# yanielc/medical-vision-textural-bias

Hardware: AMD Instinct MI355X
Metric: BraTS 4ch 240^3 vols/sec filtered+train-step @1/2/4/8 GPU; filter HBM GB/s (higher is better)
Workload: dtype f32

## Files before the change

### medical-vision-textural-bias_amd/csrc/conv_small.hip

```cpp
#include <hip/hip_runtime.h>

#include <cstdlib>

#include "texbias.h"
#include "kernels.h"

namespace {

constexpr int NT = 256;
constexpr int ROWS = 6;
constexpr int WPT = 4;
constexpr int kSeg = 3;

template <int CI, int CO>
__global__ __launch_bounds__(NT) void k_conv3d_small(const float* __restrict__ x, const float* __restrict__ wt,
                                                     const float* __restrict__ bias, float* __restrict__ y, int D,
                                                     int H, int W, int XP, int nhb) {
  extern __shared__ __attribute__((aligned(16))) float xs[];
  static_assert(WPT == 4, "the input reads are one float4 + one float2");
  float* ws = xs + CI * 3 * (ROWS + 2) * XP;
  const int tid = (int)threadIdx.x;
  for (int i = tid; i < CO * CI * 27; i += NT) ws[i] = wt[i];
  const int hb = (int)blockIdx.x % nhb, z = (int)blockIdx.x / nhb, n = (int)blockIdx.y;
  const int h0 = hb * ROWS;
  const int64_t plane = (int64_t)H * W, vol = (int64_t)D * plane;
  constexpr int NR = CI * 3 * (ROWS + 2);
  const int lane = tid & 63, wave = __builtin_amdgcn_readfirstlane(tid >> 6);
  static_assert(NR % (NT / 64) == 0, "rows deal evenly to the waves");
#pragma unroll
  for (int row = wave; row < NR; row += NT / 64) {
    const int ci = row / (3 * (ROWS + 2)), rem = row - ci * (3 * (ROWS + 2));
    const int tz = rem / (ROWS + 2), r = rem - tz * (ROWS + 2);
    const int zi = z + tz - 1, hi = h0 + r - 1;
    const bool ok = zi >= 0 && zi < D && hi >= 0 && hi < H;
    const float* src = x + ((int64_t)n * CI + ci) * vol + (ok ? (int64_t)zi * plane + (int64_t)hi * W : 0) - 1;
    float* dst = xs + row * XP;
#pragma unroll
    for (int sg = 0; sg < kSeg; ++sg) {
      const int col = lane + 64 * sg;
      const bool in = ok && col >= 1 && col <= W;
      const float v = src[in ? col : 1];
      if (col < XP) dst[col] = in ? v : 0.f;
    }
  }
  __syncthreads();
  const int tpr = (W + WPT - 1) / WPT;
  const int r = tid / tpr, w0 = (tid - r * tpr) * WPT;
  if (r >= ROWS || h0 + r >= H) return;
  float acc[CO][WPT];
#pragma unroll
  for (int co = 0; co < CO; ++co) {
    const float b = bias ? bias[co] : 0.f;
#pragma unroll
    for (int k = 0; k < WPT; ++k) acc[co][k] = b;
  }
#pragma unroll 1
  for (int ct = 0; ct < CI * 3; ++ct) {
    const int ci = ct / 3, tz = ct - 3 * ci;
    {
#pragma unroll
      for (int ty = 0; ty < 3; ++ty) {
        const float* src = xs + (ct * (ROWS + 2) + r + ty) * XP + w0;
        const float4 v4 = *reinterpret_cast<const float4*>(src);
        const float2 v2 = *reinterpret_cast<const float2*>(src + 4);
        const float v[WPT + 2] = {v4.x, v4.y, v4.z, v4.w, v2.x, v2.y};
#pragma unroll
        for (int co = 0; co < CO; ++co) {
#pragma unroll
          for (int tx = 0; tx < 3; ++tx) {
            const float wv = ws[(((co * CI + ci) * 3 + tz) * 3 + ty) * 3 + tx];
#pragma unroll
            for (int k = 0; k < WPT; ++k) acc[co][k] = fmaf(wv, v[k + tx], acc[co][k]);
          }
        }
      }
    }
  }
  const int h = h0 + r;
#pragma unroll
  for (int co = 0; co < CO; ++co) {
    float* dst = y + ((int64_t)n * CO + co) * vol + (int64_t)z * plane + (int64_t)h * W + w0;
#pragma unroll
    for (int k = 0; k < WPT; ++k)
      if (w0 + k < W) dst[k] = acc[co][k];
  }
}

typedef __attribute__((address_space(1))) const void* gptr_t;
typedef __attribute__((address_space(3))) void* lptr_t;
#ifndef TB_SMALL_ZB
#define TB_SMALL_ZB 8
#endif
constexpr int ZB = TB_SMALL_ZB;

#ifndef TB_SMALL_SW
#define TB_SMALL_SW 1
#endif
typedef const __attribute__((address_space(4))) float* cfloat_sp;

template <int CI, int CO, bool ADD = false, int U = 1>
__global__ __launch_bounds__(NT) void k_conv3d_small_z(const float* __restrict__ x, const float* __restrict__ wt,
                                                       const float* __restrict__ bias, float* __restrict__ y, int D,
                                                       int H, int W, int XP, int nhb, const float* __restrict__ add) {
  extern __shared__ __attribute__((aligned(16))) float xs[];
  constexpr int RS = ROWS + 2, NR = CI * RS;
  const int slot_f = CI * RS * XP;
  float* ws = xs + 4 * slot_f;
  const int tid = (int)threadIdx.x, lane = tid & 63, wave = __builtin_amdgcn_readfirstlane(tid >> 6);
  for (int i = tid; i < 4 * slot_f; i += NT) xs[i] = 0.f;
  for (int i = tid; i < CO * CI * 27; i += NT) ws[i] = wt[i];
  const int hb = (int)blockIdx.x % nhb, z0 = ((int)blockIdx.x / nhb) * ZB, n = (int)blockIdx.y;
  const int h0 = hb * ROWS;
  const int64_t plane = (int64_t)H * W, vol = (int64_t)D * plane;
  __syncthreads();
  auto stage = [&](int zi) {
    float* sl = xs + ((zi - z0 + 1) & 3) * slot_f;
    for (int row = wave; row < NR; row += NT / 64) {
      const int ci = row / RS, r = row - ci * RS, hi = h0 + r - 1;
      float* dst = sl + row * XP + 1;
      if (zi >= 0 && zi < D && hi >= 0 && hi < H) {
        const float* src = x + ((int64_t)n * CI + ci) * vol + (int64_t)zi * plane + (int64_t)hi * W;
#pragma unroll
        for (int sg = 0; sg < kSeg; ++sg) {
          const int c = lane + 64 * sg;
          if (c < W) __builtin_amdgcn_global_load_lds((gptr_t)(src + c), (lptr_t)(dst + 64 * sg), 4, 0, 0);
        }
      } else {
#pragma unroll
        for (int sg = 0; sg < kSeg; ++sg) {
          const int c = lane + 64 * sg;
          if (c < W) dst[c] = 0.f;
        }
      }
    }
  };
  stage(z0 - 1);
  stage(z0);
  stage(z0 + 1);
  __builtin_amdgcn_s_waitcnt(0);
  __syncthreads();
  const int tpr = (W + WPT - 1) / WPT;
  const int r = tid / tpr, w0 = (tid - r * tpr) * WPT;
  const bool act = r < ROWS && h0 + r < H;
  const int zend = z0 + ZB < D ? z0 + ZB : D;
  const int h = h0 + r;
  float prev[CO][WPT], padd[CO][WPT];
  auto put = [&](int zp) {
#pragma unroll
    for (int co = 0; co < CO; ++co) {
      const int64_t o = ((int64_t)n * CO + co) * vol + (int64_t)zp * plane + (int64_t)h * W + w0;
#pragma unroll
      for (int k = 0; k < WPT; ++k)
        if (w0 + k < W) y[o + k] = ADD ? prev[co][k] + padd[co][k] : prev[co][k];
    }
  };
  for (int z = z0; z < zend; ++z) {
    if (z + 2 < zend + 1) stage(z + 2);
    if (act) {
      if (z > z0) put(z - 1);
      if (ADD) {
#pragma unroll
        for (int co = 0; co < CO; ++co) {
          const int64_t o = ((int64_t)n * CO + co) * vol + (int64_t)z * plane + (int64_t)h * W + w0;
#pragma unroll
          for (int k = 0; k < WPT; ++k) padd[co][k] = w0 + k < W ? add[o + k] : 0.f;
        }
      }
      float acc[CO][WPT];
#pragma unroll
      for (int co = 0; co < CO; ++co) {
        const float b = bias ? bias[co] : 0.f;
#pragma unroll
        for (int k = 0; k < WPT; ++k) acc[co][k] = b;
      }
#pragma unroll U
      for (int ct = 0; ct < CI * 3; ++ct) {
        const int ci = ct / 3, tz = ct - 3 * ci;
        const float* base = xs + ((z - z0 + tz) & 3) * slot_f + (ci * RS + r) * XP + w0;
#pragma unroll
        for (int ty = 0; ty < 3; ++ty) {
          const float* src = base + ty * XP;
          const float4 v4 = *reinterpret_cast<const float4*>(src);
          const float2 v2 = *reinterpret_cast<const float2*>(src + 4);
          const float v[WPT + 2] = {v4.x, v4.y, v4.z, v4.w, v2.x, v2.y};
#pragma unroll
          for (int co = 0; co < CO; ++co) {
#pragma unroll
            for (int tx = 0; tx < 3; ++tx) {
              const int wi = (((co * CI + ci) * 3 + tz) * 3 + ty) * 3 + tx;
              const float wv = TB_SMALL_SW ? ((cfloat_sp)wt)[wi] : ws[wi];
#pragma unroll
              for (int k = 0; k < WPT; ++k) acc[co][k] = fmaf(wv, v[k + tx], acc[co][k]);
            }
          }
        }
      }
#pragma unroll
      for (int co = 0; co < CO; ++co)
#pragma unroll
        for (int k = 0; k < WPT; ++k) prev[co][k] = acc[co][k];
    }
    __builtin_amdgcn_s_waitcnt(0);
    __syncthreads();
  }
  if (act && zend > z0) put(zend - 1);
}

__global__ __launch_bounds__(256) void k_add_inplace(float* __restrict__ y, const float* __restrict__ a, int64_t n) {
  for (int64_t i = (int64_t)blockIdx.x * 256 + threadIdx.x; i < n; i += (int64_t)gridDim.x * 256) y[i] += a[i];
}

template <int CI, int CO>
int launch(const float* x, const float* w, const float* b, const float* add, float* y, int N, int D, int H, int W,
           hipStream_t st) {
  const int XP = (W + 2 + WPT + 3) / 4 * 4;
  const size_t lds = sizeof(float) * ((size_t)CI * 3 * (ROWS + 2) * XP + CO * CI * 27);
  if ((W + WPT - 1) / WPT * ROWS > NT || lds > 65536 || XP > 64 * kSeg) return TB_ERR_UNSUPPORTED_SIZE;
  const int nhb = (H + ROWS - 1) / ROWS;
  const size_t lds_z = sizeof(float) * ((size_t)4 * CI * (ROWS + 2) * XP + CO * CI * 27);
  if (lds_z <= 65536 * 2) {
    void (*kern)(const float*, const float*, const float*, float*, int, int, int, int, int, const float*) =
        add ? k_conv3d_small_z<CI, CO, true, 3> : k_conv3d_small_z<CI, CO, false, 3>;
    if (tb::allow_full_lds(kern) != hipSuccess) return TB_ERR_HIP;
    hipLaunchKernelGGL(kern, dim3((unsigned)(nhb * ((D + ZB - 1) / ZB)), (unsigned)N), dim3(NT), lds_z, st, x, w, b, y,
                       D, H, W, XP, nhb, add);
    return hipGetLastError() == hipSuccess ? TB_OK : TB_ERR_HIP;
  }
  hipLaunchKernelGGL((k_conv3d_small<CI, CO>), dim3((unsigned)(nhb * D), (unsigned)N), dim3(NT), lds, st, x, w, b, y,
                     D, H, W, XP, nhb);
  if (add) {
    const int64_t n = (int64_t)N * CO * D * H * W;
    hipLaunchKernelGGL(k_add_inplace, dim3((unsigned)((n + 1023) / 1024 < 8192 ? (n + 1023) / 1024 : 8192)), dim3(256),
                       0, st, y, add, n);
  }
  return hipGetLastError() == hipSuccess ? TB_OK : TB_ERR_HIP;
}

}

int tb_conv3d_small_f32(const float* x, const float* w, const float* b, float* y, int N, int Cin, int Cout, int D,
                        int H, int W, void* stream) {
  return tb_conv3d_small_add_f32(x, w, b, nullptr, y, N, Cin, Cout, D, H, W, stream);
}

int tb_conv3d_small_add_f32(const float* x, const float* w, const float* b, const float* add, float* y, int N, int Cin,
                            int Cout, int D, int H, int W, void* stream) {
  if (!x || !w || !y || N < 1 || D < 1 || H < 1 || W < 1 || N > 65535) return TB_ERR_INVALID_ARG;
  if (Cin < 1 || Cin > 4 || Cout < 1 || Cout > 4) return TB_ERR_UNSUPPORTED_SIZE;
  hipStream_t st = reinterpret_cast<hipStream_t>(stream);
#define TB_CASE(ci, co) \
  if (Cin == ci && Cout == co) return launch<ci, co>(x, w, b, add, y, N, D, H, W, st);
#define TB_ROW(ci) TB_CASE(ci, 1) TB_CASE(ci, 2) TB_CASE(ci, 3) TB_CASE(ci, 4)
  TB_ROW(1) TB_ROW(2) TB_ROW(3) TB_ROW(4)
#undef TB_ROW
#undef TB_CASE
  return TB_ERR_UNSUPPORTED_SIZE;
}
```

### medical-vision-textural-bias_amd/csrc/conv_up.hip

```cpp
#include <hip/hip_runtime.h>

#include <cstdlib>

#include "num_cu.h"
#include "texbias.h"

namespace {

typedef float f2v __attribute__((ext_vector_type(2)));
typedef float f32x4 __attribute__((ext_vector_type(4)));
typedef const __attribute__((address_space(4))) float* cfloat_p;
typedef const __attribute__((address_space(4))) f2v* cf2v_p;

struct S2Args {
  const float* in;
  const float* K;
  const float* bias;
  float* out;
  int Do, Ho, Wo, Di, Hi, Wi;
  int ZS, zlen, nyb;
  int PX, RR;
};

template <int CIN, int MOUT, int TY, int WV, int NTH = 256>
__global__ __launch_bounds__(NTH) void k_conv_s2_fewin(S2Args a) {
  static_assert(MOUT % 2 == 0, "packed output pairs");
  constexpr int NHALF = NTH / 256, MP = MOUT / 2 / NHALF;
  constexpr int NR = 2 * TY + 1;
  extern __shared__ __attribute__((aligned(16))) float smem[];
  const int tid = (int)threadIdx.x;
  constexpr int PX = 4 * WV + 12, SS = CIN * NR * PX;
  float* ring = smem;
  for (int i = tid; i < 3 * SS; i += NTH) ring[i] = 0.f;
  int b = (int)blockIdx.x;
  const int zs = b % a.ZS;
  b /= a.ZS;
  const int yb = b % a.nyb, n = b / a.nyb;
  const int y0 = yb * TY;
  const int z0 = zs * a.zlen, z1 = min(a.Do, z0 + a.zlen);
  const int Di = a.Di, Hi = a.Hi, Wi = a.Wi;
  const int64_t iplane = (int64_t)Hi * Wi, iplane4 = iplane / 4;
  const float4* inb = reinterpret_cast<const float4*>(a.in + (int64_t)n * CIN * Di * iplane);
  const int W4 = Wi >> 2;
  constexpr int NL = (CIN * NR * WV + NTH - 1) / NTH;
  int gof[NL], lof[NL];
#pragma unroll
  for (int j = 0; j < NL; ++j) {
    const int i = tid + NTH * j;
    const int q = i % W4, t = i / W4, r = t % NR, c = t / NR;
    const int yi = 2 * y0 - 1 + r;
    const bool ok = c < CIN && yi >= 0 && yi < Hi;
    gof[j] = ok ? (int)((int64_t)c * Di * iplane4 + ((int64_t)yi * Wi + 4 * q) / 4) : -1;
    lof[j] = (c * NR + r) * PX + 4 + 4 * q;
  }
  float4 ra[NL], rb[NL];
  auto load = [&](int zi, float4 (&r)[NL]) {
    const bool in = zi >= 0 && zi < Di;
    const float4* src = inb + (int64_t)(in ? zi : 0) * iplane4;
#pragma unroll
    for (int j = 0; j < NL; ++j) {
      r[j] = src[gof[j] < 0 ? 0 : gof[j]];
    }
  };
  auto store = [&](int zi, const float4 (&r)[NL]) {
    float* d = ring + ((zi + 3) % 3) * SS;
    const bool in = zi >= 0 && zi < Di;
#pragma unroll
    for (int j = 0; j < NL; ++j)
      if (gof[j] >= 0) *reinterpret_cast<float4*>(d + lof[j]) = in ? r[j] : make_float4(0.f, 0.f, 0.f, 0.f);
  };
  __syncthreads();
  load(2 * z0 - 1, ra);
  store(2 * z0 - 1, ra);
  load(2 * z0, ra);
  load(2 * z0 + 1, rb);
  const int pt = tid & 255, mh = __builtin_amdgcn_readfirstlane(tid >> 8);
  const int Wo = a.Wo, oy = pt / Wo, ox = pt - oy * Wo;
  const bool act = oy < TY && y0 + oy < a.Ho;
  const int roff = (2 * oy) * PX + 2 * ox + 3;
  f2v bias2[MP];
#pragma unroll
  for (int mm = 0; mm < MP; ++mm) {
    const int m = mh * MP + mm;
    bias2[mm] = a.bias ? f2v{a.bias[2 * m], a.bias[2 * m + 1]} : f2v{0.f, 0.f};
  }
  const int64_t oplane = (int64_t)a.Ho * Wo;
  float* outb = a.out + (int64_t)n * MOUT * a.Do * oplane + (int64_t)(y0 + oy) * Wo + ox;
  constexpr bool LATE = NTH == 256;
  f2v pend[MP];
  auto put = [&](int zp) {
    float* o = outb + (int64_t)zp * oplane;
#pragma unroll
    for (int mm = 0; mm < MP; ++mm) {
      const int m = mh * MP + mm;
      o[(int64_t)(2 * m) * a.Do * oplane] = pend[mm].x;
      o[(int64_t)(2 * m + 1) * a.Do * oplane] = pend[mm].y;
    }
  };
  for (int z = z0; z < z1; ++z) {
    store(2 * z, ra);
    store(2 * z + 1, rb);
    __syncthreads();
    if (LATE || z + 1 < z1) {
      load(2 * z + 2, ra);
      load(2 * z + 3, rb);
    }
    if (LATE && act && z > z0) put(z - 1);
    if (act) {
      float v[CIN * 27];
#pragma unroll
      for (int tz = 0; tz < 3; ++tz) {
        const float* sl = ring + ((2 * z - 1 + tz + 3) % 3) * SS + roff;
#pragma unroll
        for (int c = 0; c < CIN; ++c)
#pragma unroll
          for (int ty = 0; ty < 3; ++ty)
#pragma unroll
            for (int tx = 0; tx < 3; ++tx) v[c * 27 + tz * 9 + ty * 3 + tx] = sl[(c * NR + ty) * PX + tx];
      }
      const cf2v_p kp = (cf2v_p)(cfloat_p)a.K;
#pragma unroll
      for (int mm = 0; mm < MP; ++mm) {
        const int m = mh * MP + mm;
        f2v acc = bias2[mm];
#pragma unroll
        for (int k = 0; k < CIN * 27; ++k) acc = __builtin_elementwise_fma(f2v{v[k], v[k]}, kp[m * CIN * 27 + k], acc);
        if (LATE) {
          pend[mm] = acc;
        } else {
          float* o = outb + (int64_t)z * oplane;
          o[(int64_t)(2 * m) * a.Do * oplane] = acc.x;
          o[(int64_t)(2 * m + 1) * a.Do * oplane] = acc.y;
        }
      }
    }
    __syncthreads();
  }
  if (LATE && act && z1 > z0) put(z1 - 1);
}

struct TArgs {
  const float* x;
  const float* W;
  const float* bias;
  float* y;
  int Cin, Di, Hi, Wi;
  int ZS, zlen, nyb;
  int PX, CS;
};

template <int MO, int TY, int WV, int NTH = 256, int U = 1>
__global__ __launch_bounds__(NTH) void k_convT_fewout(TArgs a) {
  extern __shared__ __attribute__((aligned(16))) float smem[];
  const int tid = (int)threadIdx.x;
  constexpr int PX = 4 * WV + 8, CS = (TY + 1) * PX;
  const int Cin = a.Cin, SS = Cin * CS;
  float* ring = smem;
  for (int i = tid; i < 2 * SS; i += NTH) ring[i] = 0.f;
  const cfloat_p wg = (cfloat_p)a.W;
  int b = (int)blockIdx.x;
  const int zs = b % a.ZS;
  b /= a.ZS;
  const int yb = b % a.nyb, n = b / a.nyb;
  const int y0 = yb * TY;
  const int Di = a.Di, Hi = a.Hi, Wi = a.Wi;
  const int z0 = zs * a.zlen, z1 = min(Di, z0 + a.zlen);
  const int64_t iplane = (int64_t)Hi * Wi, iplane4 = iplane / 4;
  const float4* xb = reinterpret_cast<const float4*>(a.x + (int64_t)n * Cin * Di * iplane);
  const int W4 = Wi >> 2;
  constexpr int NL = (32 * (TY + 1) * WV + NTH - 1) / NTH;
  const int nitem = Cin * (TY + 1) * W4;
  int gof[NL], lof[NL];
#pragma unroll
  for (int j = 0; j < NL; ++j) {
    const int i = tid + NTH * j;
    const int q = i % W4, t = i / W4, r = t % (TY + 1), c = t / (TY + 1);
    const int yi = y0 + r;
    const bool ok = i < nitem && yi < Hi;
    gof[j] = ok ? (int)((int64_t)c * Di * iplane4 + ((int64_t)yi * Wi + 4 * q) / 4) : -1;
    lof[j] = c * CS + r * PX + 4 + 4 * q;
  }
  float4 rg[NL];
  auto load = [&](int zi) {
    const bool in = zi < Di;
    const float4* src = xb + (int64_t)(in ? zi : 0) * iplane4;
#pragma unroll
    for (int j = 0; j < NL; ++j) {
      rg[j] = src[gof[j] < 0 ? 0 : gof[j]];
    }
  };
  auto store = [&](int zi) {
    float* d = ring + (zi & 1) * SS;
    const bool in = zi < Di;
#pragma unroll
    for (int j = 0; j < NL; ++j)
      if (gof[j] >= 0) *reinterpret_cast<float4*>(d + lof[j]) = in ? rg[j] : make_float4(0.f, 0.f, 0.f, 0.f);
  };
  __syncthreads();
  load(z0);
  store(z0);
  load(z0 + 1);
  const int jy = tid / Wi, jx = tid - jy * Wi;
  const bool act = jy < TY && y0 + jy < Hi;
  const int roff = jy * PX + jx + 4;
  const int Ho = 2 * Hi, Wo = 2 * Wi, Do = 2 * Di;
  const int64_t oplane = (int64_t)Ho * Wo;
  float bia[MO];
#pragma unroll
  for (int m = 0; m < MO; ++m) bia[m] = a.bias ? a.bias[m] : 0.f;
  float* yb0 = a.y + (int64_t)n * MO * Do * oplane + (int64_t)(2 * (y0 + jy)) * Wo + 2 * jx;
  for (int z = z0; z < z1; ++z) {
    store(z + 1);
    __syncthreads();
    if (z + 1 < z1) load(z + 2);
    float acc[MO][2][2][2];
#pragma unroll
    for (int m = 0; m < MO; ++m)
#pragma unroll
      for (int p = 0; p < 8; ++p) acc[m][p >> 2][(p >> 1) & 1][p & 1] = bia[m];
    if (act) {
      const float* s0 = ring + (z & 1) * SS + roff;
      const float* s1 = ring + ((z + 1) & 1) * SS + roff;
#pragma unroll U
      for (int c = 0; c < Cin; ++c) {
        float v[2][2][2];
        v[0][0][0] = s0[c * CS];
        v[0][0][1] = s0[c * CS + 1];
        v[0][1][0] = s0[c * CS + PX];
        v[0][1][1] = s0[c * CS + PX + 1];
        v[1][0][0] = s1[c * CS];
        v[1][0][1] = s1[c * CS + 1];
        v[1][1][0] = s1[c * CS + PX];
        v[1][1][1] = s1[c * CS + PX + 1];
        const cfloat_p wc = wg + c * MO * 27;
#pragma unroll
        for (int m = 0; m < MO; ++m) {
          const cfloat_p wk = wc + m * 27;
#pragma unroll
          for (int pz = 0; pz < 2; ++pz)
#pragma unroll
            for (int py = 0; py < 2; ++py)
#pragma unroll
              for (int px = 0; px < 2; ++px) {
                float s = acc[m][pz][py][px];
#pragma unroll
                for (int dz = 0; dz <= pz; ++dz)
#pragma unroll
                  for (int dy = 0; dy <= py; ++dy)
#pragma unroll
                    for (int dx = 0; dx <= px; ++dx) {
                      const int tz = pz ? (dz ? 0 : 2) : 1, ty = py ? (dy ? 0 : 2) : 1, tx = px ? (dx ? 0 : 2) : 1;
                      s = fmaf(v[dz][dy][dx], wk[tz * 9 + ty * 3 + tx], s);
                    }
                acc[m][pz][py][px] = s;
              }
        }
      }
#pragma unroll
      for (int m = 0; m < MO; ++m)
#pragma unroll
        for (int pz = 0; pz < 2; ++pz)
#pragma unroll
          for (int py = 0; py < 2; ++py) {
            float* o = yb0 + ((int64_t)m * Do + 2 * z + pz) * oplane + (int64_t)py * Wo;
            *reinterpret_cast<float2*>(o) = make_float2(acc[m][pz][py][0], acc[m][pz][py][1]);
          }
    }
    __syncthreads();
  }
}

int zseg(int D, int base, int per_cu, int fill) {
  const int slots = per_cu * tb::num_cu();
  int best = 1 << 30, zl = D;
  for (int l = D; l >= 1; --l) {
    const int zs = (D + l - 1) / l, rounds = (base * zs + slots - 1) / slots, cost = rounds * (l + fill);
    if (cost < best) best = cost, zl = l;
  }
  return zl;
}

template <int CIN, int MOUT, int WV>
int launch_s2(S2Args& a, size_t lds, int N, hipStream_t st) {
  constexpr int TY = 3;
  constexpr int NT = (CIN == 4 && MOUT == 32) ? 512 : 256;
  auto kern = k_conv_s2_fewin<CIN, MOUT, TY, WV, NT>;
  if (hipFuncSetAttribute(reinterpret_cast<const void*>(kern), hipFuncAttributeMaxDynamicSharedMemorySize, 163840) !=
      hipSuccess)
    return TB_ERR_HIP;
  const int per_cu = lds <= 81920 ? 2 : 1;
  a.zlen = zseg(a.Do, N * a.nyb, per_cu, 1);
  a.ZS = (a.Do + a.zlen - 1) / a.zlen;
  hipLaunchKernelGGL(kern, dim3((unsigned)(N * a.nyb * a.ZS)), dim3(NT), lds, st, a);
  return hipGetLastError() == hipSuccess ? TB_OK : TB_ERR_HIP;
}

}

int tb_conv3d_s2_fewin_f32(const float* in, const float* K, const float* bias, float* out, int N, int Cin, int Mout,
                           int Do, int Ho, int Wo, void* stream) {
  if (!in || !K || !out || N < 1 || Do < 1 || Ho < 1 || Wo < 1) return TB_ERR_INVALID_ARG;
  if (Cin < 1 || Cin > 4 || (Mout != 16 && Mout != 32) || 3 * Wo > 256 || (2 * Wo) % 4 != 0 || 2 * Wo > 256 ||
      (reinterpret_cast<uintptr_t>(in) & 15) != 0)
    return TB_ERR_UNSUPPORTED_SIZE;
  constexpr int TY = 3;
  S2Args a{};
  a.in = in, a.K = K, a.bias = bias, a.out = out;
  a.Do = Do, a.Ho = Ho, a.Wo = Wo, a.Di = 2 * Do, a.Hi = 2 * Ho, a.Wi = 2 * Wo;
  const bool wide = a.Wi > 160;
  a.PX = 4 * (wide ? 64 : 40) + 12;
  a.RR = 2 * TY + 1;
  a.nyb = (Ho + TY - 1) / TY;
  const size_t lds = (size_t)4 * 3 * Cin * a.RR * a.PX;
  if (lds > 163840) return TB_ERR_UNSUPPORTED_SIZE;
  hipStream_t st = reinterpret_cast<hipStream_t>(stream);
#define TB_S2(CI, MO)                                                                                  \
  if (Cin == CI && Mout == MO) return wide ? launch_s2<CI, MO, 64>(a, lds, N, st) : launch_s2<CI, MO, 40>(a, lds, N, st);
  TB_S2(1, 16) TB_S2(2, 16) TB_S2(3, 16) TB_S2(4, 16) TB_S2(1, 32) TB_S2(2, 32) TB_S2(3, 32) TB_S2(4, 32)
#undef TB_S2
  return TB_ERR_UNSUPPORTED_SIZE;
}

int tb_convT3d_fewout_f32(const float* x, const float* W, const float* bias, float* y, int N, int Cin, int Mout, int Di,
                          int Hi, int Wi, void* stream) {
  if (!x || !W || !y || N < 1 || Di < 1 || Hi < 1 || Wi < 1) return TB_ERR_INVALID_ARG;
  if (Cin < 1 || Cin > 32 || Mout < 1 || Mout > 4 || Wi % 4 != 0 || Wi > 128 || (reinterpret_cast<uintptr_t>(x) & 15) != 0)
    return TB_ERR_UNSUPPORTED_SIZE;
  const bool big = Wi <= 80 && (size_t)4 * 2 * Cin * 7 * (4 * 20 + 8) <= 163840;
  const int TY = big ? 6 : 256 / Wi >= 3 ? 3 : 256 / Wi >= 2 ? 2 : 1;
  const int nth = big ? 512 : 256;
  TArgs a{};
  a.x = x, a.W = W, a.bias = bias, a.y = y;
  a.Cin = Cin, a.Di = Di, a.Hi = Hi, a.Wi = Wi;
  a.PX = 4 * (Wi <= 80 ? 20 : 32) + 8;
  a.CS = (TY + 1) * a.PX;
  a.nyb = (Hi + TY - 1) / TY;
  const size_t lds = (size_t)4 * 2 * Cin * a.CS;
  if (lds > 163840) return TB_ERR_UNSUPPORTED_SIZE;
  const int per_cu = lds <= 81920 ? 2 : 1;
  a.zlen = zseg(Di, N * a.nyb, per_cu, 1);
  a.ZS = (Di + a.zlen - 1) / a.zlen;
  hipStream_t st = reinterpret_cast<hipStream_t>(stream);
  const dim3 grid((unsigned)(N * a.nyb * a.ZS));
  void (*kern)(TArgs) = nullptr;
#define TB_T(MO, T)                                                                    \
  if (Mout == MO && TY == T) kern = Wi <= 80 ? k_convT_fewout<MO, T, 20> : k_convT_fewout<MO, T, 32>;
  TB_T(1, 1) TB_T(1, 2) TB_T(1, 3) TB_T(2, 1) TB_T(2, 2) TB_T(2, 3) TB_T(3, 1) TB_T(3, 2) TB_T(3, 3) TB_T(4, 1)
  TB_T(4, 2) TB_T(4, 3)
#undef TB_T
  constexpr int U = 1;
  if (big && Mout == 3)
    kern = U == 4 ? k_convT_fewout<3, 6, 20, 512, 4> : U == 2 ? k_convT_fewout<3, 6, 20, 512, 2>
                                                      : k_convT_fewout<3, 6, 20, 512>;
  else if (big)
    kern = Mout == 1 ? k_convT_fewout<1, 6, 20, 512> : Mout == 2 ? k_convT_fewout<2, 6, 20, 512>
                                                     : k_convT_fewout<4, 6, 20, 512>;
  if (!kern) return TB_ERR_UNSUPPORTED_SIZE;
  if (hipFuncSetAttribute(reinterpret_cast<const void*>(kern), hipFuncAttributeMaxDynamicSharedMemorySize, 163840) !=
      hipSuccess)
    return TB_ERR_HIP;
  hipLaunchKernelGGL(kern, grid, dim3(nth), lds, st, a);
  return hipGetLastError() == hipSuccess ? TB_OK : TB_ERR_HIP;
}

namespace {
struct F16Args {
  const float* x;
  const float* W;
  const float* bias;
  const float* add;
  float* y;
  int D, H, Wd;
  int ZS, zlen, nyb;
  int PX, RX;
  int flip;
  int persist, ncol;
  int64_t addsn;
};

template <int YB, int NXT, int NTH, bool ADD = false, bool PF = false, int NS = 3>
__global__ __launch_bounds__(NTH) void k_conv3d_fwd16(F16Args a) {
  constexpr int NWV = NTH / 64;
  extern __shared__ __attribute__((aligned(16))) float smem[];
  constexpr int NR = YB + 2, W4 = 4 * NXT;
  const int tid = (int)threadIdx.x, lane = tid & 63;
  const int wave = __builtin_amdgcn_readfirstlane(tid >> 6);
  const int D = a.D, H = a.H, Wd = a.Wd, PX = a.PX, RX = a.RX, SS = 16 * RX;
  float* ring = smem;
  for (int i = tid; i < NS * SS; i += NTH) ring[i] = 0.f;
  const int li = lane & 15, ks = lane >> 4;
  float af[108];
#pragma unroll
  for (int kk = 0; kk < 108; ++kk) {
    const int c = 4 * (kk & 3) + ks, t = kk >> 2;
    af[kk] = a.flip ? a.W[(c * 16 + li) * 27 + 26 - t] : a.W[(li * 16 + c) * 27 + t];
  }
  const float bm[4] = {a.bias ? a.bias[4 * ks] : 0.f, a.bias ? a.bias[4 * ks + 1] : 0.f,
                       a.bias ? a.bias[4 * ks + 2] : 0.f, a.bias ? a.bias[4 * ks + 3] : 0.f};
  int64_t s_beg, s_end;
  if (a.persist) {
    const int64_t T = (int64_t)a.ncol * D;
    s_beg = T * blockIdx.x / gridDim.x, s_end = T * (blockIdx.x + 1) / gridDim.x;
  } else {
    int b = (int)blockIdx.x;
    const int zs = b % a.ZS;
    b /= a.ZS;
    const int zb = zs * a.zlen;
    s_beg = (int64_t)b * D + zb, s_end = (int64_t)b * D + min(D, zb + a.zlen);
  }
  for (int64_t sg = s_beg; sg < s_end;) {
  const int col = (int)(sg / D), z0 = (int)(sg - (int64_t)col * D);
  const int z1 = (int)min((int64_t)D, z0 + (s_end - sg));
  sg += z1 - z0;
  const int yb = col % a.nyb, n = col / a.nyb;
  const int y0 = yb * YB;
  const int64_t plane = (int64_t)H * Wd, plane4 = plane / 4;
  const float4* xb = reinterpret_cast<const float4*>(a.x + (int64_t)n * 16 * D * plane);
  constexpr int NL = (16 * NR * W4 + NTH - 1) / NTH;
  int gof[NL], lof[NL];
#pragma unroll
  for (int j = 0; j < NL; ++j) {
    const int i = tid + NTH * j;
    const int q = i % W4, t = i / W4, r = t % NR, c = t / NR;
    const int yi = y0 - 1 + r;
    const bool ok = i < 16 * NR * W4 && yi >= 0 && yi < H;
    gof[j] = ok ? (int)((int64_t)c * D * plane4 + ((int64_t)yi * Wd + 4 * q) / 4) : -1;
    lof[j] = i < 16 * NR * W4 ? c * RX + r * PX + 4 + 4 * q : 0;
  }
  float4 rg[NL];
  auto load = [&](int zi) {
    const bool in = zi >= 0 && zi < D;
    const float4* src = xb + (int64_t)(in ? zi : 0) * plane4;
#pragma unroll
    for (int j = 0; j < NL; ++j) {
      rg[j] = src[gof[j] < 0 ? 0 : gof[j]];
    }
  };
// ... 613 lines not shown
```

Before: 170.1.

## Register-staged z-pipeline, software-pipelined weight loads, fused residual, adaptive z-blocking

```diff
diff --git a/medical-vision-textural-bias_amd/csrc/conv_small.hip b/medical-vision-textural-bias_amd/csrc/conv_small.hip
--- a/medical-vision-textural-bias_amd/csrc/conv_small.hip
+++ b/medical-vision-textural-bias_amd/csrc/conv_small.hip
@@ -4,6 +4,7 @@
 
 #include "texbias.h"
 #include "kernels.h"
+#include "num_cu.h"
 
 namespace {
 
@@ -86,128 +87,186 @@
   }
 }
 
-typedef __attribute__((address_space(1))) const void* gptr_t;
-typedef __attribute__((address_space(3))) void* lptr_t;
 #ifndef TB_SMALL_ZB
-#define TB_SMALL_ZB 8
+#define TB_SMALL_ZB 0
 #endif
 constexpr int ZB = TB_SMALL_ZB;
-
-#ifndef TB_SMALL_SW
-#define TB_SMALL_SW 1
-#endif
+constexpr int NS = 3;
 typedef const __attribute__((address_space(4))) float* cfloat_sp;
-
-template <int CI, int CO, bool ADD = false, int U = 1>
+typedef float f4v __attribute__((ext_vector_type(4)));
+typedef float f2v __attribute__((ext_vector_type(2)));
+
+template <int CI, int CO, int RES = 0>
 __global__ __launch_bounds__(NT) void k_conv3d_small_z(const float* __restrict__ x, const float* __restrict__ wt,
                                                        const float* __restrict__ bias, float* __restrict__ y, int D,
-                                                       int H, int W, int XP, int nhb, const float* __restrict__ add) {
+                                                       int H, int W, int XP, int nhb, const float* __restrict__ add,
+                                                       int vec, int zb) {
+  static_assert(RES != 2 || CI == CO, "the aliased residual is the input itself");
   extern __shared__ __attribute__((aligned(16))) float xs[];
-  constexpr int RS = ROWS + 2, NR = CI * RS;
+  constexpr int RS = ROWS + 2, NR = CI * RS, NW = NT / 64;
+  constexpr int NJ = NR / NW;
+  constexpr int NG = CI * 3, GW = CO * 9;
+  static_assert(NR % NW == 0, "rows deal evenly to the waves");
   const int slot_f = CI * RS * XP;
-  float* ws = xs + 4 * slot_f;
   const int tid = (int)threadIdx.x, lane = tid & 63, wave = __builtin_amdgcn_readfirstlane(tid >> 6);
-  for (int i = tid; i < 4 * slot_f; i += NT) xs[i] = 0.f;
-  for (int i = tid; i < CO * CI * 27; i += NT) ws[i] = wt[i];
-  const int hb = (int)blockIdx.x % nhb, z0 = ((int)blockIdx.x / nhb) * ZB, n = (int)blockIdx.y;
+  for (int i = tid; i < NS * slot_f / 4; i += NT)
+    reinterpret_cast<f4v*>(xs)[i] = f4v{0.f, 0.f, 0.f, 0.f};
+  const int hb = (int)blockIdx.x % nhb, z0 = ((int)blockIdx.x / nhb) * zb, n = (int)blockIdx.y;
   const int h0 = hb * ROWS;
   const int64_t plane = (int64_t)H * W, vol = (int64_t)D * plane;
+  const int zend = z0 + zb < D ? z0 + zb : D;
+  static_assert(RS == 2 * NW, "a wave's rows: two per channel");
+  int hoff[2], cof[kSeg], lcol[kSeg];
+  unsigned lm[2][kSeg];
+#pragma unroll
+  for (int q = 0; q < 2; ++q) {
+    const int hi = h0 + wave + NW * q - 1;
+#pragma unroll
+    for (int sg = 0; sg < kSeg; ++sg) lm[q][sg] = ((hi >= 0) & (hi < H) & (lane + 64 * sg < W)) ? ~0u : 0u;
+    hoff[q] = (hi < 0 ? 0 : hi >= H ? H - 1 : hi) * W;
+  }
+#pragma unroll
+  for (int sg = 0; sg < kSeg; ++sg) {
+    cof[sg] = lane + 64 * sg < W ? lane + 64 * sg : W - 1;
+    lcol[sg] = lane + 64 * sg < W ? lane + 64 * sg : XP - 2;
+  }
+  const float* xn = x + (int64_t)n * CI * vol;
+  auto load = [&](int zi, float (&rg)[NJ][kSeg]) {
+    const bool need = zi <= zend;
+    const float* xz = xn + (need ? (int64_t)(zi < 0 ? 0 : zi >= D ? D - 1 : zi) * plane : 0);
+    const int64_t cv = need ? vol : 0;
+    const int nm = need ? ~0 : 0;
+#pragma unroll
+    for (int j = 0; j < NJ; ++j) {
+      const float* src = xz + (int64_t)(j >> 1) * cv + (hoff[j & 1] & nm);
+#pragma unroll
+      for (int sg = 0; sg < kSeg; ++sg) rg[j][sg] = src[cof[sg] & nm];
+    }
+  };
+  auto store = [&](int zi, const float (&rg)[NJ][kSeg]) {
+    float* sl = xs + ((zi - z0 + 1) % NS) * slot_f + 1;
+    const unsigned zm = ((zi >= 0) & (zi < D)) ? ~0u : 0u;
+#pragma unroll
+    for (int j = 0; j < NJ; ++j) {
+      float* dst = sl + (wave + NW * j) * XP;
+#pragma unroll
+      for (int sg = 0; sg < kSeg; ++sg)
+        dst[lcol[sg]] = __uint_as_float(__float_as_uint(rg[j][sg]) & lm[j & 1][sg] & zm);
+    }
+  };
+  float ra[NJ][kSeg], rb[NJ][kSeg], rc[NJ][kSeg];
   __syncthreads();
-  auto stage = [&](int zi) {
-    float* sl = xs + ((zi - z0 + 1) & 3) * slot_f;
-    for (int row = wave; row < NR; row += NT / 64) {
-      const int ci = row / RS, r = row - ci * RS, hi = h0 + r - 1;
-      float* dst = sl + row * XP + 1;
-      if (zi >= 0 && zi < D && hi >= 0 && hi < H) {
-        const float* src = x + ((int64_t)n * CI + ci) * vol + (int64_t)zi * plane + (int64_t)hi * W;
-#pragma unroll
-        for (int sg = 0; sg < kSeg; ++sg) {
-          const int c = lane + 64 * sg;
-          if (c < W) __builtin_amdgcn_global_load_lds((gptr_t)(src + c), (lptr_t)(dst + 64 * sg), 4, 0, 0);
-        }
-      } else {
-#pragma unroll
-        for (int sg = 0; sg < kSeg; ++sg) {
-          const int c = lane + 64 * sg;
-          if (c < W) dst[c] = 0.f;
-        }
-      }
-    }
-  };
-  stage(z0 - 1);
-  stage(z0);
-  stage(z0 + 1);
-  __builtin_amdgcn_s_waitcnt(0);
+  load(z0 - 1, ra);
+  load(z0, rb);
+  load(z0 + 1, rc);
+  store(z0 - 1, ra);
+  store(z0, rb);
+  store(z0 + 1, rc);
   __syncthreads();
   const int tpr = (W + WPT - 1) / WPT;
   const int r = tid / tpr, w0 = (tid - r * tpr) * WPT;
   const bool act = r < ROWS && h0 + r < H;
-  const int zend = z0 + ZB < D ? z0 + ZB : D;
   const int h = h0 + r;
-  float prev[CO][WPT], padd[CO][WPT];
+  float bv[CO];
+#pragma unroll
+  for (int co = 0; co < CO; ++co) bv[co] = bias ? bias[co] : 0.f;
+  const cfloat_sp wc = (cfloat_sp)wt;
+  auto issue = [&](int g, int zr, float (&wg)[GW], float (&vg)[3][WPT + 2]) {
+    const int ci = g / 3, tz = g - 3 * ci;
+#pragma unroll
+    for (int co = 0; co < CO; ++co)
+#pragma unroll
+      for (int t = 0; t < 9; ++t) wg[co * 9 + t] = wc[((co * CI + ci) * 3 + tz) * 9 + t];
+    const float* base = xs + ((zr + tz) % NS) * slot_f + (ci * RS + r) * XP + w0;
+#pragma unroll
+    for (int ty = 0; ty < 3; ++ty) {
+      const f4v v4 = *reinterpret_cast<const f4v*>(base + ty * XP);
+      const f2v v2 = *reinterpret_cast<const f2v*>(base + ty * XP + 4);
+      vg[ty][0] = v4.x, vg[ty][1] = v4.y, vg[ty][2] = v4.z, vg[ty][3] = v4.w, vg[ty][4] = v2.x, vg[ty][5] = v2.y;
+    }
+  };
+  float prev[CO][WPT];
   auto put = [&](int zp) {
 #pragma unroll
     for (int co = 0; co < CO; ++co) {
-      const int64_t o = ((int64_t)n * CO + co) * vol + (int64_t)zp * plane + (int64_t)h * W + w0;
-#pragma unroll
-      for (int k = 0; k < WPT; ++k)
-        if (w0 + k < W) y[o + k] = ADD ? prev[co][k] + padd[co][k] : prev[co][k];
+      float* o = y + ((int64_t)n * CO + co) * vol + (int64_t)zp * plane + (int64_t)h * W + w0;
+      if (vec) {
+        *reinterpret_cast<f4v*>(o) = f4v{prev[co][0], prev[co][1], prev[co][2], prev[co][3]};
+      } else {
+#pragma unroll
+        for (int k = 0; k < WPT; ++k)
+          if (w0 + k < W) o[k] = prev[co][k];
+      }
     }
   };
   for (int z = z0; z < zend; ++z) {
-    if (z + 2 < zend + 1) stage(z + 2);
+    load(z + 2, ra);
     if (act) {
-      if (z > z0) put(z - 1);
-      if (ADD) {
+      float res[CO][WPT];
+      if (RES == 1) {
 #pragma unroll
         for (int co = 0; co < CO; ++co) {
-          const int64_t o = ((int64_t)n * CO + co) * vol + (int64_t)z * plane + (int64_t)h * W + w0;
-#pragma unroll
-          for (int k = 0; k < WPT; ++k) padd[co][k] = w0 + k < W ? add[o + k] : 0.f;
+          const float* s = add + ((int64_t)n * CO + co) * vol + (int64_t)z * plane + (int64_t)h * W + w0;
+#pragma unroll
+          for (int k = 0; k < WPT; ++k) res[co][k] = s[w0 + k < W ? k : 0];
         }
       }
+      if (z > z0) put(z - 1);
       float acc[CO][WPT];
 #pragma unroll
-      for (int co = 0; co < CO; ++co) {
-        const float b = bias ? bias[co] : 0.f;
-#pragma unroll
-        for (int k = 0; k < WPT; ++k) acc[co][k] = b;
+      for (int co = 0; co < CO; ++co)
+#pragma unroll
+        for (int k = 0; k < WPT; ++k) acc[co][k] = bv[co];
+      float wg[2][GW], vg[2][3][WPT + 2];
+      issue(0, z - z0, wg[0], vg[0]);
+#pragma unroll
+      for (int g = 0; g < NG; ++g) {
+        const int ci = g / 3, tz = g - 3 * ci;
+        __builtin_amdgcn_sched_barrier(0);
+        __builtin_amdgcn_s_waitcnt(0xc07f);
+        __builtin_amdgcn_sched_barrier(0);
+        if (g + 1 < NG) issue(g + 1, z - z0, wg[(g + 1) & 1], vg[(g + 1) & 1]);
+        __builtin_amdgcn_sched_barrier(0);
+        const float(&w)[GW] = wg[g & 1];
+        const float(&v)[3][WPT + 2] = vg[g & 1];
+#pragma unroll
+        for (int ty = 0; ty < 3; ++ty)
+#pragma unroll
+          for (int co = 0; co < CO; ++co)
+#pragma unroll
+            for (int tx = 0; tx < 3; ++tx)
+#pragma unroll
+              for (int k = 0; k < WPT; ++k) acc[co][k] = fmaf(w[co * 9 + ty * 3 + tx], v[ty][k + tx], acc[co][k]);
+        if (RES == 2 && tz == 1) {
+#pragma unroll
+          for (int k = 0; k < WPT; ++k) res[ci < CO ? ci : 0][k] = v[1][k + 1];
+        }
+        __builtin_amdgcn_sched_barrier(0);
       }
-#pragma unroll U
-      for (int ct = 0; ct < CI * 3; ++ct) {
-        const int ci = ct / 3, tz = ct - 3 * ci;
-        const float* base = xs + ((z - z0 + tz) & 3) * slot_f + (ci * RS + r) * XP + w0;
-#pragma unroll
-        for (int ty = 0; ty < 3; ++ty) {
-          const float* src = base + ty * XP;
-          const float4 v4 = *reinterpret_cast<const float4*>(src);
-          const float2 v2 = *reinterpret_cast<const float2*>(src + 4);
-          const float v[WPT + 2] = {v4.x, v4.y, v4.z, v4.w, v2.x, v2.y};
-#pragma unroll
-          for (int co = 0; co < CO; ++co) {
-#pragma unroll
-            for (int tx = 0; tx < 3; ++tx) {
-              const int wi = (((co * CI + ci) * 3 + tz) * 3 + ty) * 3 + tx;
-              const float wv = TB_SMALL_SW ? ((cfloat_sp)wt)[wi] : ws[wi];
-#pragma unroll
-              for (int k = 0; k < WPT; ++k) acc[co][k] = fmaf(wv, v[k + tx], acc[co][k]);
-            }
-          }
-        }
-      }
 #pragma unroll
       for (int co = 0; co < CO; ++co)
 #pragma unroll
-        for (int k = 0; k < WPT; ++k) prev[co][k] = acc[co][k];
-    }
-    __builtin_amdgcn_s_waitcnt(0);
+        for (int k = 0; k < WPT; ++k) prev[co][k] = RES ? acc[co][k] + res[co][k] : acc[co][k];
+    }
     __syncthreads();
-  }
-  if (act && zend > z0) put(zend - 1);
+    store(z + 2, ra);
+    __syncthreads();
+  }
+  if (act) put(zend - 1);
 }
 
 __global__ __launch_bounds__(256) void k_add_inplace(float* __restrict__ y, const float* __restrict__ a, int64_t n) {
   for (int64_t i = (int64_t)blockIdx.x * 256 + threadIdx.x; i < n; i += (int64_t)gridDim.x * 256) y[i] += a[i];
+}
+
+int zplanes(int D, int base, int per_cu) {
+  const int slots = (per_cu < 1 ? 1 : per_cu) * tb::num_cu();
+  int best = 1 << 30, zl = D;
+  for (int l = D; l >= (D < 8 ? D : 8); --l) {
+    const int zs = (D + l - 1) / l, rounds = (base * zs + slots - 1) / slots, cost = rounds * (l + 2);
+    if (cost < best) best = cost, zl = l;
+  }
+  return zl;
 }
 
 template <int CI, int CO>
@@ -215,15 +274,21 @@
            hipStream_t st) {
   const int XP = (W + 2 + WPT + 3) / 4 * 4;
   const size_t lds = sizeof(float) * ((size_t)CI * 3 * (ROWS + 2) * XP + CO * CI * 27);
-  if ((W + WPT - 1) / WPT * ROWS > NT || lds > 65536 || XP > 64 * kSeg) return TB_ERR_UNSUPPORTED_SIZE;
+  if ((W + WPT - 1) / WPT * ROWS > NT || lds > 65536 || XP > 64 * kSeg || (int64_t)H * W > (1 << 29))
+    return TB_ERR_UNSUPPORTED_SIZE;
   const int nhb = (H + ROWS - 1) / ROWS;
-  const size_t lds_z = sizeof(float) * ((size_t)4 * CI * (ROWS + 2) * XP + CO * CI * 27);
+  const size_t lds_z = sizeof(float) * ((size_t)NS * CI * (ROWS + 2) * XP);
   if (lds_z <= 65536 * 2) {
-    void (*kern)(const float*, const float*, const float*, float*, int, int, int, int, int, const float*) =
-        add ? k_conv3d_small_z<CI, CO, true, 3> : k_conv3d_small_z<CI, CO, false, 3>;
+    void (*kern)(const float*, const float*, const float*, float*, int, int, int, int, int, const float*, int, int) =
+        k_conv3d_small_z<CI, CO, 0>;
+    if (add) kern = k_conv3d_small_z<CI, CO, 1>;
+    if constexpr (CI == CO)
+      if (add == x) kern = k_conv3d_small_z<CI, CO, 2>;
     if (tb::allow_full_lds(kern) != hipSuccess) return TB_ERR_HIP;
-    hipLaunchKernelGGL(kern, dim3((unsigned)(nhb * ((D + ZB - 1) / ZB)), (unsigned)N), dim3(NT), lds_z, st, x, w, b, y,
-                       D, H, W, XP, nhb, add);
+    const int vec = W % 4 == 0 && (reinterpret_cast<uintptr_t>(y) & 15) == 0;
+    const int zb = ZB ? ZB : zplanes(D, N * nhb, (int)(163840 / lds_z));
+    hipLaunchKernelGGL(kern, dim3((unsigned)(nhb * ((D + zb - 1) / zb)), (unsigned)N), dim3(NT), lds_z, st, x, w, b, y,
+                       D, H, W, XP, nhb, add, vec, zb);
     return hipGetLastError() == hipSuccess ? TB_OK : TB_ERR_HIP;
   }
   hipLaunchKernelGGL((k_conv3d_small<CI, CO>), dim3((unsigned)(nhb * D), (unsigned)N), dim3(NT), lds, st, x, w, b, y,
diff --git a/medical-vision-textural-bias_amd/csrc/conv_up.hip b/medical-vision-textural-bias_amd/csrc/conv_up.hip
--- a/medical-vision-textural-bias_amd/csrc/conv_up.hip
+++ b/medical-vision-textural-bias_amd/csrc/conv_up.hip
@@ -1,6 +1,7 @@
 #include <hip/hip_runtime.h>
 
 #include <cstdlib>
+#include <type_traits>
 
 #include "num_cu.h"
 #include "texbias.h"
@@ -11,6 +12,14 @@
 typedef float f32x4 __attribute__((ext_vector_type(4)));
 typedef const __attribute__((address_space(4))) float* cfloat_p;
 typedef const __attribute__((address_space(4))) f2v* cf2v_p;
+
+template <int B, int N, class F>
+__device__ __forceinline__ void static_for(F&& f) {
+  if constexpr (B < N) {
+    f(std::integral_constant<int, B>{});
+    static_for<B + 1, N>(f);
+  }
+}
 
 struct S2Args {
   const float* in;
@@ -118,21 +127,42 @@
 #pragma unroll
             for (int tx = 0; tx < 3; ++tx) v[c * 27 + tz * 9 + ty * 3 + tx] = sl[(c * NR + ty) * PX + tx];
       }
-      const cf2v_p kp = (cf2v_p)(cfloat_p)a.K;
-#pragma unroll
-      for (int mm = 0; mm < MP; ++mm) {
-        const int m = mh * MP + mm;
-        f2v acc = bias2[mm];
-#pragma unroll
-        for (int k = 0; k < CIN * 27; ++k) acc = __builtin_elementwise_fma(f2v{v[k], v[k]}, kp[m * CIN * 27 + k], acc);
-        if (LATE) {
-          pend[mm] = acc;
-        } else {
-          float* o = outb + (int64_t)z * oplane;
-          o[(int64_t)(2 * m) * a.Do * oplane] = acc.x;
-          o[(int64_t)(2 * m + 1) * a.Do * oplane] = acc.y;
+      constexpr int KC = CIN * 27, NP = MP * KC, BT = 16, NB = (NP + BT - 1) / BT;
+      const cf2v_p kp = (cf2v_p)(cfloat_p)a.K + mh * NP;
+      f2v kb[2][BT];
+      auto kload = [&](int b, f2v (&k)[BT]) {
+#pragma unroll
+        for (int i = 0; i < BT; ++i)
+          if (b * BT + i < NP) k[i] = kp[b * BT + i];
+      };
+      kload(0, kb[0]);
+      f2v acc = bias2[0];
+      static_for<0, NB>([&](auto bc) {
+        constexpr int b = decltype(bc)::value;
+        __builtin_amdgcn_sched_barrier(0);
+        __builtin_amdgcn_s_waitcnt(0xc07f);
+        __builtin_amdgcn_sched_barrier(0);
+        if (b + 1 < NB) kload(b + 1, kb[(b + 1) & 1]);
+        __builtin_amdgcn_sched_barrier(0);
+#pragma unroll
+        for (int i = 0; i < BT; ++i) {
+          const int p = b * BT + i, mm = p / KC, k = p - mm * KC;
+          if (p < NP) {
+            if (k == 0) acc = bias2[mm];
+            acc = __builtin_elementwise_fma(f2v{v[k], v[k]}, kb[b & 1][i], acc);
+            if (k == KC - 1) {
+              if (LATE) {
+                pend[mm] = acc;
+              } else {
+                const int m = mh * MP + mm;
+                float* o = outb + (int64_t)z * oplane;
+                o[(int64_t)(2 * m) * a.Do * oplane] = acc.x;
+                o[(int64_t)(2 * m + 1) * a.Do * oplane] = acc.y;
+              }
+            }
+          }
         }
-      }
+      });
     }
     __syncthreads();
   }
```

Result: faster. 173.8 (median of 6 runs) (+2.2%).
